# rasoolims/ImageTranslate

Measured on AMD Instinct MI355X. Metric: train tokens/sec (whole node), 6L enc-dec d=512 seq128 b64, 1/2/4/8 GPU, higher is better.
Workload: dtype bf16; 1 GPU; 6L/6L enc-dec d=512 h=8 ff=2048 V=30000, src[64,128] tgt[64,128], synthetic random-token MT; global_batch=64, seq_len=128, parallelism=dp1, distinct_batches=8, directions=2

## Files before the change

imagetranslate_amd/_lib.py:

```python
import ctypes
import os
from ctypes import POINTER, Structure, c_char_p, c_float, c_int, c_int32, c_int64, c_uint64, c_void_p

_HERE = os.path.dirname(os.path.abspath(__file__))
LIB_PATH = os.environ.get("IMT_LIB") or os.path.join(_HERE, "libimt_hip.so")

IMT_F32, IMT_BF16 = 0, 1
IMT_NT, IMT_NN, IMT_TN = 0, 1, 2
IMT_AUX_NONE, IMT_AUX_GELU_FWD, IMT_AUX_DGELU, IMT_AUX_SPLITK_WS = 0, 1, 2, 3


class GemmArgs(Structure):
    _fields_ = [
        ("dtype", c_int32), ("layout", c_int32),
        ("M", c_int32), ("N", c_int32), ("K", c_int32),
        ("A", c_void_p), ("lda", c_int64),
        ("B", c_void_p), ("ldb", c_int64),
        ("C", c_void_p), ("ldc", c_int64),
        ("c_dtype", c_int32), ("accumulate", c_int32),
        ("bias", c_void_p),
        ("resid", c_void_p), ("ldr", c_int64),
        ("aux", c_void_p), ("ldaux", c_int64),
        ("aux_mode", c_int32), ("split_k", c_int32),
        ("alpha", c_float), ("dropout_p", c_float),
# ... 172 lines not shown
        ("dtype", c_int32), ("B", c_int32), ("S", c_int32), ("T", c_int32), ("d", c_int32),
        ("x", c_void_p), ("ldx", c_int64), ("bsx", c_int64),
        ("y", c_void_p), ("ldy", c_int64), ("bsy", c_int64),
        ("xr", c_void_p), ("yr", c_void_p),
        ("min_sim", c_float), ("reserved", c_int32),
        ("link", c_void_p), ("fwd_idx", c_void_p), ("fwd_val", c_void_p), ("bwd_idx", c_void_p), ("bwd_val", c_void_p),
    ]


_P = c_void_p
SIGNATURES = {
    "imt_version": (c_int, []),
    "imt_last_error": (c_char_p, []),
    "imt_gemm": (c_int, [POINTER(GemmArgs), _P]),
    "imt_gemm_grouped_tn": (c_int, [POINTER(GemmArgs), c_int, _P]),
    "imt_gemm_splitk_ws_bytes": (c_int64, []),
    "imt_gemm_bias_residual_ln_supported": (c_int, [c_int, c_int, c_int]),
    "imt_gemm_bias_residual_ln": (c_int, [c_int, _P, c_int64, _P, c_int64, _P, _P, c_int64, _P, _P, _P, _P, c_int64, _P, _P, c_int, c_int,
                                          c_int, c_float, c_float, c_uint64, _P]),
    "imt_colsum": (c_int, [c_int, _P, c_int64, c_int, c_int, _P, _P, _P]),
    "imt_layernorm_fwd": (c_int, [c_int, _P, _P, _P, _P, _P, _P, c_int, c_int, c_float, c_float, c_uint64, _P]),
    "imt_add_layernorm_fwd": (c_int, [c_int, _P, _P, _P, _P, _P, _P, _P, _P, c_int, c_int, c_float, c_float, c_uint64, _P]),
    "imt_embed_ln_fwd": (c_int, [c_int, _P, _P, _P, _P, _P, _P, _P, _P, _P, _P, _P, _P, c_int, c_int, c_int, c_int, c_int, c_int, c_float,
                                 c_float, c_uint64, _P]),
    "imt_layernorm_bwd": (c_int, [c_int, _P, _P, _P, _P, _P, _P, _P, _P, c_int, c_int, c_float, c_uint64, _P, c_float,
                                  c_uint64, _P, _P]),
    "imt_embed_fwd": (c_int, [c_int, _P, _P, _P, _P, _P, _P, _P, c_int, c_int, c_int, c_int, c_int, c_int, _P]),
    "imt_embed_bwd": (c_int, [c_int, _P, _P, _P, _P, _P, _P, _P, c_int, c_int, c_int, c_int64, _P]),
    "imt_attention_fwd": (c_int, [POINTER(AttnArgs), _P]),
    "imt_attention_bwd": (c_int, [POINTER(AttnArgs), _P]),
# ... 38 lines not shown
    "imt_l2_dist": (c_int, [c_int, _P, _P, _P, _P, _P, c_int, c_int64, _P]),
    "imt_sensim_loss": (c_int, [_P, _P, _P, _P, _P, _P, c_int, c_int, c_int, c_int, _P]),
    "imt_pair_dot": (c_int, [_P, _P, _P, c_int64, c_int, _P]),
    "imt_pair_dot_bwd": (c_int, [_P, _P, _P, _P, _P, c_int64, c_int, _P]),
    "imt_proposal_attn_ws_bytes": (c_int64, [c_int64, c_int, c_int, c_int]),
    "imt_proposal_attn_fwd": (c_int, [c_int, _P, _P, _P, _P, _P, _P, _P, _P, _P, c_int64, c_int, c_int, c_int, c_int64, c_int64, c_float, _P]),
    "imt_proposal_attn_bwd": (c_int, [c_int, _P, _P, _P, _P, _P, _P, _P, _P, _P, _P, _P, _P, _P, _P, c_int64, c_int64, c_int, c_int, c_int,
                                      c_int64, c_int64, _P]),
    "imt_comm_unique_id_bytes": (c_int, []),
    "imt_comm_get_unique_id": (c_int, [_P]),
    "imt_comm_init": (c_int, [_P, c_int, c_int, POINTER(c_void_p)]),
    "imt_comm_allreduce": (c_int, [_P, _P, c_int64, c_int, _P]),
    "imt_comm_broadcast": (c_int, [_P, _P, c_int64, c_int, c_int, _P]),
    "imt_comm_destroy": (c_int, [_P]),
    "imt_set_gemm_share_cus": (c_int, [c_int]),
    "imt_debug_spin": (c_int, [c_int, c_int, c_int, c_int64, _P]),
    "imt_abi_sizeof": (c_int, [ctypes.c_char_p]),
    "imt_prof_enable": (c_int, [c_int]),
    "imt_prof_report": (c_int, [POINTER(ProfRow), c_int]),
    "imt_stack_workspace_bytes": (c_int64, [POINTER(StackDesc), c_int, c_int, c_int]),
    "imt_stack_forward": (c_int, [POINTER(StackDesc), POINTER(StackIO), _P, c_int64, _P]),
    "imt_stack_backward": (c_int, [POINTER(StackDesc), POINTER(StackIO), _P, c_int64, c_int, c_int, _P]),
    "imt_attention_decode": (c_int, [POINTER(AttnDecodeArgs), _P]),
    "imt_decode_workspace_bytes": (c_int64, [POINTER(StackDesc), c_int]),
    "imt_decode_self_cache_bytes": (c_int64, [POINTER(StackDesc), c_int, c_int]),
    "imt_decode_cross_bytes": (c_int64, [POINTER(StackDesc), c_int, c_int]),
    "imt_decode_begin": (c_int, [POINTER(StackDesc), _P, c_int, c_int, _P, _P]),
    "imt_decode_step": (c_int, [POINTER(StackDesc), POINTER(DecodeIO), _P, c_int64, _P]),
    "imt_decode_check": (c_int, [POINTER(StackDesc), c_int, _P, _P]),
    "imt_beam_step": (c_int, [POINTER(BeamArgs), _P]),
# ... 48 lines not shown
```

imagetranslate_amd/csrc/common.hpp:

```cpp
#pragma once
#include <hip/hip_runtime.h>
#include <stdint.h>
#include <stdio.h>
#include <string.h>
#include "../../include/imt_hip.h"

typedef __bf16 bf16_t;
typedef __attribute__((ext_vector_type(4))) float f32x4;
typedef __attribute__((ext_vector_type(2))) float f32x2;
typedef __attribute__((ext_vector_type(8))) __bf16 bf16x8;
typedef __attribute__((ext_vector_type(4))) __bf16 bf16x4;
typedef __attribute__((ext_vector_type(2))) __bf16 bf16x2;
typedef __attribute__((ext_vector_type(4))) short s16x4;
typedef __attribute__((ext_vector_type(4))) unsigned int u32x4;
typedef __attribute__((ext_vector_type(2))) unsigned int u32x2;

#define IMT_WAVE 64
#define IMT_DEVICE __device__ __forceinline__

void imt_set_error(const char* fmt, ...);

#define IMT_CHECK_ARG(cond, ...)                       \
  do {                                                  \
    if (!(cond)) {                                      \
// ... 8 lines not shown
    if (e__ != hipSuccess) {                                                 \
      imt_set_error("%s:%d launch failed: %s", __FILE__, __LINE__,           \
                    hipGetErrorString(e__));                                 \
      return IMT_ERR_LAUNCH;                                                 \
    }                                                                        \
  } while (0)

static inline int imt_cdiv(long a, long b) { return (int)((a + b - 1) / b); }
static inline bool imt_ok_dtype(int t) { return t == IMT_F32 || t == IMT_BF16; }
static inline int imt_dtype_bytes(int t) { return t == IMT_BF16 ? 2 : 4; }
static inline int64_t imt_align256(int64_t bytes) { return (bytes + 255) / 256 * 256; }
template <typename T> struct ImtType { typedef T type; };
template <typename F> static inline int imt_by_dtype(int dtype, F&& f) {
  return dtype == IMT_F32 ? f(ImtType<float>()) : f(ImtType<bf16_t>());
}

bool imt_prof_enabled();
const char* imt_prof_intern(const char* kind, int M, int N, int K);
void* imt_prof_begin_launch(const char* kind, double flops, double bytes, hipStream_t st);
void imt_prof_end_launch(void* tok, hipStream_t st);
#include <stdlib.h>
struct ImtTrace {
  static constexpr int MAXB = 4096;
  static constexpr int RING = 64;
  unsigned long long* dev = nullptr;
  const char* kind; int blocks; hipStream_t st;
  struct Slot { const char* kind; int blocks; };
  static Slot* slots() { static Slot s[RING]; return s; }
  static int& count() { static int c = 0; return c; }
  static bool ring() { static const bool r = getenv("IMT_TRACE_RING") != nullptr; return r; }
// ... 239 lines not shown
```

imagetranslate_amd/csrc/gemm.hip:

```cpp
#include <stdlib.h>
#include "mma.hpp"
#include "gemm_xl.hpp"

namespace {

constexpr int BM = 128, BN = 128, NTHREADS = 256;
constexpr int STAGE_BYTES = 2 * TILE_BYTES;


template <typename T, bool KCONTIG> struct Stage : TileGeom<T, KCONTIG> {
  using G = TileGeom<T, KCONTIG>;
  u32x4 r[4];
  IMT_DEVICE void load(const T* __restrict__ base, int64_t ld, int row0, int nrows, int k0, int K) {
    const int tid = threadIdx.x;
#pragma unroll
    for (int i = 0; i < 4; ++i) {
      const int q = i * NTHREADS + tid;
      const int tr = q / G::CPR, c = q % G::CPR;
      int64_t grow, gcol;
      bool ok;
      if (KCONTIG) { grow = row0 + tr; gcol = k0 + c * G::EPC; ok = (grow < nrows) && (gcol < K); }
      else         { grow = k0 + tr;   gcol = row0 + c * G::EPC; ok = (grow < K) && (gcol < nrows); }
      u32x4 v = {0u, 0u, 0u, 0u};
      if (ok) v = *reinterpret_cast<const u32x4*>(base + grow * ld + gcol);
// ... 689 lines not shown
      if (LAYOUT == IMT_TN && do_colsum) cs.flush(smem + half * 16384, ep.a_colsum, m0 + 128 * half, M, alpha, true, ht);
      return;
    }
  }
#pragma unroll 1
  for (int q = 0; q < 4; ++q) {
    const int qm = q >> 1, qn = q & 1;
    const int mq = m0 + 128 * qm, nq = n0 + 128 * qn;
    if (mq >= M || nq >= N) continue;
    if (wmi == qm && (wni >> 1) == qn) epilogue<T, XL_THREADS, true, 128>(acc, smem, mq, nq, 0, wn, M, N, ep, alpha);
    else                               epilogue<T, XL_THREADS, false, 128>(acc, smem, mq, nq, 0, wn, M, N, ep, alpha);
  }
  if (LAYOUT == IMT_TN && do_colsum) cs.flush(smem + half * 16384, ep.a_colsum, m0 + 128 * half, M, alpha, true, ht);
}

constexpr int MAX_GROUP = 8;
struct GroupProblem {
  const void* A; const void* B; float* C; float* a_colsum;
  int64_t lda, ldb, ldc, a_bytes, b_bytes;
  int M, N, K, tile_start;
};
struct GroupArgs { int count; int total_tiles; float alpha; int alpha_pad_order ; GroupProblem p[MAX_GROUP]; };

constexpr int GROUP_NST = 4;
constexpr int GROUP_THREADS = 512;

template <typename T> IMT_DEVICE typename Frag<T>::type ones_frag();
template <> IMT_DEVICE f32x4 ones_frag<float>() { return f32x4{1.f, 1.f, 1.f, 1.f}; }
template <> IMT_DEVICE bf16x8 ones_frag<bf16_t>() {
  const bf16_t o = (bf16_t)1.0f;
  return bf16x8{o, o, o, o, o, o, o, o};
}

template <typename T, bool CS, bool LO>
IMT_DEVICE void grouped_consumer_loop(f32x4 (&acc)[4][4], f32x4 (&bacc)[2], const char* smem, int nt, int wm, int wn) {
  typedef typename Frag<T>::type frag_t;
  constexpr int MPF = sizeof(T) == 2 ? 1 : 4;
// ... 23 lines not shown
#pragma unroll
    for (int i = 0; i < 4; ++i)
#pragma unroll
      for (int j = 0; j < 4; ++j) mma16(acc[i][j], f1b[j], f1a[i]);
    if (CS) { mma16(bacc[0], ones, f1a[LO ? 0 : 2]); mma16(bacc[1], ones, f1a[LO ? 1 : 3]); }
#pragma unroll
    for (int k = 0; k < 16; ++k) {
      __builtin_amdgcn_sched_group_barrier(0x008, MPF, 0);
      __builtin_amdgcn_sched_group_barrier(0x100, 1, 0);
    }
    __builtin_amdgcn_sched_barrier(0);
    cur = nxt;
  }
}

template <typename T>
__global__ __launch_bounds__(GROUP_THREADS) void gemm_grouped_tn_kernel(GroupArgs g) {
  constexpr int BK = TileGeom<T, false>::BK;
  extern __shared__ __attribute__((aligned(16))) char smem[];
  const int bid = (g.alpha_pad_order == 0) ? imt_xcd_block(blockIdx.x, g.total_tiles) : (int)blockIdx.x;
  int pi = 0;
#pragma unroll
  for (int i = 1; i < MAX_GROUP; ++i)
    if (i < g.count && bid >= g.p[i].tile_start) pi = i;
  const GroupProblem& P = g.p[pi];
  const int M = P.M, N = P.N, K = P.K;
  const int nbx = (N + BN - 1) / BN;
  const int local = bid - P.tile_start;
  const int m0 = (local / nbx) * BM, n0 = (local % nbx) * BN;
  const int nt = (K + BK - 1) / BK;
  const int wave = __builtin_amdgcn_readfirstlane(threadIdx.x >> 6);
  const bool consumer = wave < 4;
  const int wm = ((wave & 3) >> 1) * 64, wn = (wave & 1) * 64;

  f32x4 acc[4][4];
#pragma unroll
  for (int i = 0; i < 4; ++i)
#pragma unroll
    for (int j = 0; j < 4; ++j) acc[i][j] = f32x4{0.f, 0.f, 0.f, 0.f};
  f32x4 bacc[2] = {f32x4{0.f, 0.f, 0.f, 0.f}, f32x4{0.f, 0.f, 0.f, 0.f}};
  const bool do_colsum = P.a_colsum && n0 == 0;

  if (!consumer) {
    Dma<T, false> da; Dma<T, false> db;
// ... 441 lines not shown
  int splits = a->split_k > 1 ? a->split_k : 1, kps = a->K;
  if (splits > 1) {
    IMT_CHECK_ARG(a->c_dtype == IMT_F32 && !a->bias && !a->resid && a->aux_mode == IMT_AUX_NONE && a->dropout_p == 0.f,
                  "imt_gemm: split_k supports only fp32 atomic accumulation without epilogue");
    kps = imt_cdiv(imt_cdiv(a->K, splits), f.bk) * f.bk;
    splits = imt_cdiv(a->K, kps);
  }
  if (a->aux_mode != IMT_AUX_NONE) IMT_CHECK_ARG(a->aux != nullptr, "imt_gemm: aux_mode needs aux");
  const GemmSwitches& sw = gemm_switches();
  const bool linear_epilogue = a->aux_mode == IMT_AUX_NONE && a->dropout_p == 0.f && !a->a_colsum;
  if (a->force_general == 0 && splits == 1 && a->layout != IMT_TN && a->K % f.bk != 0 && a->K / f.bk >= 16 && linear_epilogue) return run_ragged_k(a, f, stream);
  if (const int S = splitk_ws_splits(a, f, sw, splits); S > 1) return run_splitk_ws(a, f, S, stream);
  return run_single(a, f, sw, splits, kps, stream);
}

extern "C" int imt_gemm_grouped_tn(const imt_gemm_args* list, int count, void* stream) {
  IMT_CHECK_ARG(list && count >= 0, "imt_gemm_grouped_tn: bad args");
  if (count == 0) return IMT_OK;
  hipStream_t st = reinterpret_cast<hipStream_t>(stream);
  bool ok = count <= MAX_GROUP;
  const int dtype = list[0].dtype;
  const int bk = (dtype == IMT_BF16) ? 64 : 32, es = imt_dtype_bytes(dtype), al = (dtype == IMT_BF16) ? 8 : 4;
  int tiles = 0;
  for (int i = 0; i < count && ok; ++i) {
    const imt_gemm_args& a = list[i];
    ok = a.dtype == dtype && a.layout == IMT_TN && a.c_dtype == IMT_F32 && !a.bias && !a.resid && a.aux_mode == IMT_AUX_NONE &&
         a.dropout_p == 0.f && !a.alpha_dev && a.alpha == list[0].alpha && a.A && a.B && a.C && a.M > 0 && a.N > 0 &&
         a.K / bk >= 2 && a.lda % al == 0 && a.ldb % al == 0 && a.M % al == 0 && a.N % al == 0 && a.ldc % 4 == 0 &&
         (((uintptr_t)a.A | (uintptr_t)a.B) & 15) == 0 && (int64_t)a.K * a.lda * es < (1ll << 31) &&
         (int64_t)a.K * a.ldb * es < (1ll << 31);
    tiles += imt_cdiv(a.M, BM) * imt_cdiv(a.N, BN);
  }
  if (!ok || tiles > 640) {
    for (int i = 0; i < count; ++i) {
      int rc = imt_gemm(&list[i], stream);
      if (rc != IMT_OK) return rc;
    }
    return IMT_OK;
  }
  GroupArgs g;
  memset(&g, 0, sizeof(g));
  g.count = count; g.alpha = list[0].alpha; g.alpha_pad_order = gemm_switches().grouped_plain_order ? 1 : 0;
  int start = 0;
  double flops = 0, bytes = 0;
  for (int i = 0; i < count; ++i) {
    const imt_gemm_args& a = list[i];
    GroupProblem& P = g.p[i];
    P.A = a.A; P.B = a.B; P.C = reinterpret_cast<float*>(a.C); P.a_colsum = a.a_colsum;
    P.lda = a.lda; P.ldb = a.ldb; P.ldc = a.ldc;
    P.a_bytes = view_bytes(a.K, a.lda, a.M, es); P.b_bytes = view_bytes(a.K, a.ldb, a.N, es);
    P.M = a.M; P.N = a.N; P.K = a.K; P.tile_start = start;
    start += imt_cdiv(a.M, BM) * imt_cdiv(a.N, BN);
    flops += 2.0 * a.M * a.N * a.K;
    bytes += ((double)a.M + a.N) * a.K * es + 4.0 * a.M * a.N;
  }
  g.total_tiles = start;
  static const bool once_f32 = allow_lds(gemm_grouped_tn_kernel<float>, GROUP_NST * STAGE_BYTES), once_bf16 = allow_lds(gemm_grouped_tn_kernel<bf16_t>, GROUP_NST * STAGE_BYTES);
  ImtProfScope prof(dtype == IMT_BF16 ? "gemm_bf16_tn_grouped" : "gemm_f32_tn_grouped", flops, bytes, st);
  auto kern = (dtype == IMT_F32) ? gemm_grouped_tn_kernel<float> : gemm_grouped_tn_kernel<bf16_t>;
  hipLaunchKernelGGL(kern, dim3(start), dim3(GROUP_THREADS), GROUP_NST * STAGE_BYTES, st, g);
  IMT_CHECK_LAUNCH();
  return IMT_OK;
}
```

imagetranslate_amd/csrc/model.hip:

```cpp
#include "common.hpp"
#include "decode_fused.hpp"

namespace {

struct Carver {
  char* base; int64_t off;
  explicit Carver(void* b) : base(reinterpret_cast<char*>(b)), off(0) {}
  void* take(int64_t bytes) {
    void* p = base ? base + off : nullptr;
    off += (bytes + 255) & ~(int64_t)255;
    return p;
  }
};

struct AttnWs {
  void* qkv;
  void* kv;
  int64_t kv_ld;
  void* ctx;
  float* lse;
  void* pre_ln;
  float* mean; float* rstd;
  void* out;
};
// ... 2 lines not shown
  void* z; void* h;
  void* pre_ln2; float* mean2; float* rstd2;
  void* out;
};
struct StackWs {
  void* emb_sum; float* emb_mean; float* emb_rstd; void* x0;
  LayerWs* layers;
  void* d_run;
  void* dpre[3]; void* ddrop[3];
  void* d_ctx;
  void* d_ff;
  void* d_qkv;
  void* d_q;
  void* d_kv;
  void* d_emb;
  struct Scratch { void* dpre[3]; void* ddrop[3]; void* d_ctx; void* d_ff; void* d_qkv; void* d_q; void* d_kv; } scr[2];
  void use_scratch(int l) {
    const Scratch& z = scr[l & 1];
    for (int i = 0; i < 3; ++i) { dpre[i] = z.dpre[i]; ddrop[i] = z.ddrop[i]; }
    d_ctx = z.d_ctx; d_ff = z.d_ff; d_qkv = z.d_qkv; d_q = z.d_q; d_kv = z.d_kv;
  }
  void* kv_all; void* d_kv_all;
  float* delta;
  float* ln_partial;
  float* ln_site(int site, int d) const { return ln_partial + (int64_t)site * IMT_LN_BWD_WS_FLOATS(d); }
  void* splitk; int64_t splitk_bytes;
  int64_t bytes;
};

constexpr int MAX_LAYERS = 64;

int64_t kv_w_off(const imt_stack_desc* m, const imt_layer_desc& p) { return p.cross_kv_w >= 0 ? p.cross_kv_w : p.cross_attn.qkv_w + (int64_t)m->d * m->d; }
int64_t kv_b_off(const imt_stack_desc* m, const imt_layer_desc& p) { return p.cross_kv_b >= 0 ? p.cross_kv_b : p.cross_attn.qkv_b + m->d; }
// ... 29 lines not shown
    AttnWs& x = L.cross;
    memset(&x, 0, sizeof(x));
    if (m->is_decoder && m->layers[l].cross_attn.qkv_w >= 0) {
      x.qkv = c.take(N * d * es); x.ctx = c.take(N * d * es);
      if (batched) { x.kv = w.kv_all ? (void*)((char*)w.kv_all + (int64_t)l * 2 * d * es) : nullptr; x.kv_ld = L2d; }
      else { x.kv = c.take(Nk * 2 * d * es); x.kv_ld = 2 * d; }
      x.lse = (float*)c.take((int64_t)B * m->heads * T * 4);
      x.pre_ln = c.take(N * d * es); x.mean = (float*)c.take(N * 4); x.rstd = (float*)c.take(N * 4);
      x.out = c.take(N * d * es);
    }
    L.z = c.take(N * ff * es); L.h = c.take(N * ff * es);
    L.pre_ln2 = c.take(N * d * es); L.mean2 = (float*)c.take(N * 4); L.rstd2 = (float*)c.take(N * 4);
    L.out = c.take(N * d * es);
  }
  w.d_run = c.take(N * d * es);
  for (int k = 0; k < 2; ++k) {
    StackWs::Scratch& z = w.scr[k];
    for (int i = 0; i < 3; ++i) { z.dpre[i] = c.take(N * d * es); z.ddrop[i] = c.take(N * d * es); }
    z.d_ctx = c.take(N * d * es);
    z.d_ff = c.take(N * ff * es);
    z.d_qkv = c.take(N * 3 * d * es);
    z.d_q = c.take(N * d * es);
    z.d_kv = c.take((Nk > 0 ? Nk : 1) * 2 * d * es);
  }
  w.use_scratch(0);
  w.d_emb = c.take(N * d * es);
  w.delta = (float*)c.take((int64_t)B * m->heads * T * 4);
  w.ln_partial = (float*)c.take((int64_t)(3 * m->n_layers + 1) * IMT_LN_BWD_WS_FLOATS(d) * 4);
  w.splitk_bytes = ((N + 127) / 128) * ((d + 127) / 128) <= 128 ? imt_gemm_splitk_ws_bytes() : 0;
  w.splitk = w.splitk_bytes ? c.take(w.splitk_bytes) : nullptr;
  w.bytes = c.off;
// ... 46 lines not shown
                                     pre_ln, out, N, mean, rstd, M, N, K, c.m->ln_eps, drop_p, seed, c.st);
  imt_gemm_args a;
  memset(&a, 0, sizeof(a));
  a.dtype = c.dtype; a.layout = IMT_NT; a.M = M; a.N = N; a.K = K;
  a.A = x; a.lda = ldx; a.B = c.P(w_off); a.ldb = K; a.C = pre_ln; a.ldc = N; a.c_dtype = c.dtype;
  a.bias = b_off >= 0 ? c.P(b_off) : nullptr;
  a.resid = resid; a.ldr = N; a.aux_mode = IMT_AUX_NONE; a.split_k = 1; a.alpha = 1.f;
  a.dropout_p = drop_p; a.dropout_seed = seed;
  a.ln_gamma = c.P(g_off); a.ln_beta = c.P(beta_off); a.ln_out = out; a.ld_ln = N; a.ln_mean = mean; a.ln_rstd = rstd;
  a.ln_eps = c.m->ln_eps;
  a.splitk_ws = c.splitk; a.splitk_ws_bytes = c.splitk_bytes;
  return imt_gemm(&a, c.st);
}

struct DeferredDW {
  imt_gemm_args list[8];
  int n = 0;
  void add(const Ctx& c, const void* dy, int64_t lddy, const void* x, int64_t ldx, int M, int N, int K, int64_t w_off, int64_t b_off) {
    imt_gemm_args& a = list[n++];
    memset(&a, 0, sizeof(a));
    a.dtype = c.dtype; a.layout = IMT_TN; a.M = N; a.N = K; a.K = M;
    a.A = dy; a.lda = lddy; a.B = x; a.ldb = ldx; a.C = c.G(w_off); a.ldc = K; a.c_dtype = IMT_F32; a.alpha = 1.f;
    a.split_k = 1; a.accumulate = 1;
    a.a_colsum = b_off >= 0 ? c.G(b_off) : nullptr;
    const int tiles = imt_cdiv(N, 128) * imt_cdiv(K, 128);
    int sk = 1;
    while (sk < 8 && tiles * sk * 2 <= 256 && M / (sk * 2) >= 512) sk *= 2;
    if (M % (c.dtype == IMT_BF16 ? 64 : 32) != 0) { a.split_k = sk; a.accumulate = (sk == 1); }
  }
  int flush(hipStream_t st) {
    const int rc = n ? imt_gemm_grouped_tn(list, n, st) : IMT_OK;
    n = 0;
// ... 198 lines not shown
  IMT_CHECK_ARG(0 <= layer_lo && layer_lo <= layer_hi && layer_hi <= m->n_layers, "stack_backward: bad layer range");
  Ctx c{m, (hipStream_t)stream, m->dtype, imt_dtype_bytes(m->dtype)};
  c.splitk = w.splitk; c.splitk_bytes = w.splitk_bytes;
  const int B = io->B, T = io->T, N = B * T, d = m->d;
  const bool training = io->training != 0;
  const uint64_t seed = io->dropout_seed;
  const MaskSet self_ms{io->key_mask, io->query_mask, io->mask3d, io->causal};
  const MaskSet cross_ms{io->enc_mask, nullptr, nullptr, 0};
  const void* dy = (layer_hi == m->n_layers) ? io->d_out : w.d_run;
  const bool batched = cross_kv_batched(m);
  DeferredDW dw;
  const int64_t lnf = IMT_LN_BWD_WS_FLOATS(d);
  if (layer_hi > layer_lo) (void)hipMemsetAsync(w.ln_site(3 * layer_lo, d), 0, (size_t)(3 * (layer_hi - layer_lo)) * lnf * 4, c.st);
  if (layer_lo == 0) (void)hipMemsetAsync(w.ln_site(3 * m->n_layers, d), 0, (size_t)lnf * 4, c.st);
  static const bool side_env = !(getenv("IMT_DW_SIDE_STREAM") && atoi(getenv("IMT_DW_SIDE_STREAM")) == 0);
  const bool side = side_env && !imt_prof_enabled() && layer_lo == 0 && layer_hi == m->n_layers && m->n_layers >= 2 && g_side.init();
  int last_side = -1;
  for (int l = layer_hi - 1; l >= layer_lo; --l) {
    const imt_layer_desc& p = m->layers[l];
    LayerWs& L = layers[l];
    w.use_scratch(l);
    if (side && l + 2 < layer_hi) (void)hipStreamWaitEvent(c.st, g_side.done[l + 2], 0);
    if (l == m->n_layers - 1) L.out = io->out;
    const bool has_cross = m->is_decoder && p.cross_attn.qkv_w >= 0;
    const void* x_in = (l == 0) ? w.x0 : (const void*)layers[l - 1].out;
    const void* a_self = L.self_attn.out;
    const void* a_ffn_in = has_cross ? L.cross.out : a_self;
    RC(ffn_bwd(c, p, L, w, dw, a_ffn_in, N, training, seed, l, dy));
    if (has_cross) {
      const bool first_cross = (l == m->n_layers - 1);
      void* dkv_l = batched ? offp(w.d_kv_all, (int64_t)l * 2 * d, c.es) : nullptr;
      RC(attn_block_bwd(c, p.cross_attn, L.cross, w, dw, 1, a_self, B, T, io->enc_states, io->Tk, cross_ms, training, seed, l, 4, w.d_run,
                        io->d_enc_states, first_cross ? 0 : 1, kv_w_off(m, p), kv_b_off(m, p), dkv_l));
    }
    RC(attn_block_bwd(c, p.self_attn, L.self_attn, w, dw, 2, x_in, B, T, nullptr, 0, self_ms, training, seed, l, 0, w.d_run, nullptr, 0));
    if (side) {
      (void)hipEventRecord(g_side.ready[l], c.st);
      (void)hipStreamWaitEvent(g_side.st, g_side.ready[l], 0);
      RC(dw.flush(g_side.st));
      (void)hipEventRecord(g_side.done[l], g_side.st);
      last_side = l;
    } else {
      RC(dw.flush(c.st));
    }
    dy = w.d_run;
  }
  if (layer_lo == 0 && batched) {
    const int Nk = B * io->Tk;
    const int L2d = m->n_layers * 2 * d;
    if (io->d_enc_states)
      RC(linear_bwd_input(c, w.d_kv_all, L2d, Nk, L2d, m->layers[0].cross_kv_w, d, io->d_enc_states, d, nullptr, 0, nullptr, IMT_AUX_NONE, 0));
  }
  if (layer_lo == 0) {
    const void* dy0 = (m->n_layers == 0) ? io->d_out : dy;
    RC(imt_layernorm_bwd(c.dtype, dy0, w.emb_sum, c.P(m->emb_ln_g), w.emb_mean, w.emb_rstd, w.d_emb, c.G(m->emb_ln_g), c.G(m->emb_ln_b), N, d,
                         training ? m->hidden_dropout : 0.f, site_seed(seed, 1000, 0), nullptr, 0.f, 0, w.ln_site(3 * m->n_layers, d), c.st));
    RC(imt_embed_bwd(c.dtype, io->ids, io->pos_ids, io->type_ids, w.d_emb, c.G(m->emb_word), c.G(m->emb_pos), c.G(m->emb_type), N, T, d,
                     m->pad_id, c.st));
// ... 203 lines not shown
```

imagetranslate_amd/hip_ops.py:

```python
import ctypes
import os
import math

import torch

from . import _lib as L
from ._lib import IMT_AUX_DGELU, IMT_AUX_GELU_FWD, IMT_AUX_NONE, IMT_AUX_SPLITK_WS, IMT_BF16, IMT_F32, IMT_NN, IMT_NT, IMT_TN


def dt(t: torch.Tensor) -> int:
    if t.dtype == torch.float32:
        return IMT_F32
    if t.dtype == torch.bfloat16:
        return IMT_BF16
    raise TypeError("imagetranslate_amd supports float32 and bfloat16 tensors, got %s" % t.dtype)


def _stream():
    return ctypes.c_void_p(torch.cuda.current_stream().cuda_stream)


def _p(t):
    return None if t is None else ctypes.c_void_p(t.data_ptr())

# ... 73 lines not shown


def splitk_workspace(device):
    key = (device.type, device.index)
    ws = _SPLITK_WS.get(key)
    if ws is None:
        ws = torch.empty(int(L.load().imt_gemm_splitk_ws_bytes()) // 4, device=device, dtype=torch.float32)
        _SPLITK_WS[key] = ws
    return ws


def dw_split_k(rows: int, N: int, K: int, rows_per_split: int) -> int:
    return max(1, min(rows // rows_per_split, 512 // max(1, ((N + 127) // 128) * ((K + 127) // 128))))


def gemm_grouped_tn(problems):
    arr = (L.GemmArgs * len(problems))()
    for i, pr in enumerate(problems):
        arr[i] = gemm(pr["A"], pr["B"], IMT_TN, out=pr["out"], accumulate=True, a_colsum=pr.get("a_colsum"), _launch=False)
    L.check(L.load().imt_gemm_grouped_tn(arr, len(problems), _stream()), "imt_gemm_grouped_tn")


def gemm_bias_residual_ln(x, w, bias, resid, gamma, beta, eps=1e-12, dropout_p=0.0, dropout_seed=0, want_pre_ln=True):
    _req_cuda(x, w, bias, resid, gamma, beta)
    M, K = x.shape
    N = w.shape[0]
    assert w.shape[1] == K
    out = torch.empty((M, N), device=x.device, dtype=x.dtype)
    pre = torch.empty((M, N), device=x.device, dtype=x.dtype) if want_pre_ln else None
    mean = torch.empty(M, device=x.device, dtype=torch.float32)
    rstd = torch.empty(M, device=x.device, dtype=torch.float32)
    L.check(L.load().imt_gemm_bias_residual_ln(dt(x), _p(x), _rowmajor(x), _p(w), _rowmajor(w), _p(bias), _p(resid),
                                               _rowmajor(resid) if resid is not None else 0, _p(gamma), _p(beta), _p(pre), _p(out), N,
                                               _p(mean), _p(rstd), M, N, K, eps, dropout_p, dropout_seed, _stream()),
            "imt_gemm_bias_residual_ln")
# ... 775 lines not shown
```

include/imt_hip.h:

```cpp
#ifndef IMT_HIP_H
#define IMT_HIP_H
#include <stdint.h>
#ifdef __cplusplus
extern "C" {
#endif

#define IMT_OK 0
#define IMT_ERR_BAD_ARG (-1)
#define IMT_ERR_UNSUPPORTED (-2)
#define IMT_ERR_LAUNCH (-3)

#define IMT_F32 0
#define IMT_BF16 1

int imt_version(void);
const char* imt_last_error(void);

int imt_abi_sizeof(const char* struct_name);

typedef struct imt_prof_row {
  char kind[48];
  int64_t launches;
  double total_ms;
  double flops;
// ... 30 lines not shown
  const float* alpha_dev;
  float* a_colsum;
  int32_t force_general;
  int32_t force_pipeline;
  const void* ln_gamma; const void* ln_beta;
  void* ln_out; int64_t ld_ln;
  float* ln_mean; float* ln_rstd;
  int32_t* ln_tickets;
  float ln_eps;
  int32_t reserved_ln;
  void* splitk_ws; int64_t splitk_ws_bytes;
} imt_gemm_args;
int64_t imt_gemm_splitk_ws_bytes(void);
int imt_gemm(const imt_gemm_args* a, void* stream);
int imt_gemm_grouped_tn(const imt_gemm_args* list, int count, void* stream);

int imt_gemm_bias_residual_ln_supported(int dtype, int N, int K);
int imt_gemm_bias_residual_ln(int dtype, const void* x, int64_t ldx, const void* w, int64_t ldw, const void* bias,
                              const void* resid, int64_t ldr, const void* gamma, const void* beta, void* pre_ln, void* out,
                              int64_t ldo, float* mean, float* rstd, int M, int N, int K, float eps, float dropout_p,
                              uint64_t dropout_seed, void* stream);

int imt_colsum(int dtype, const void* X, int64_t ldx, int M, int N, float* out, const float* scale_dev, void* stream);

int imt_layernorm_fwd(int dtype, const void* x, const void* gamma, const void* beta, void* y, float* mean,
                      float* rstd, int rows, int d, float eps, float dropout_p, uint64_t dropout_seed,
                      void* stream);
int imt_add_layernorm_fwd(int dtype, const void* x, const void* resid, const void* gamma, const void* beta, void* sum_out,
                          void* y, float* mean, float* rstd, int rows, int d, float eps, float dropout_p,
                          uint64_t dropout_seed, void* stream);
// ... 106 lines not shown
  int32_t* fwd_idx; float* fwd_val;
  int32_t* bwd_idx; float* bwd_val;
} imt_align_args;
int imt_align_supported(int dtype, int d);
int imt_align_pairs(const imt_align_args* a, void* stream);
int imt_scaled_sum(const float* x, int n, float scale, float* out, void* stream);

int imt_comm_unique_id_bytes(void);
int imt_comm_get_unique_id(void* host_id_out);
int imt_comm_init(const void* host_unique_id, int world_size, int rank, void** comm_out);
int imt_comm_allreduce(void* comm, void* buf, int64_t count, int dtype, void* stream);
int imt_comm_broadcast(void* comm, void* buf, int64_t count, int dtype, int root, void* stream);
int imt_comm_destroy(void* comm);

int imt_set_gemm_share_cus(int share_cus);

#define IMT_SUMSQ_WS_FLOATS 1024
int imt_sumsq(const float* g, int64_t n, float* out, float* partial_ws, void* stream);
int imt_clip_adam(float* p, float* g, float* m, float* v, void* p_bf16, int64_t n, const float* sumsq,
                  float max_norm, float grad_scale, float lr, float beta1, float beta2, float eps, int64_t step,
                  int zero_grad, void* stream);
int imt_clip_scale(float* g, int64_t n, const float* sumsq, float max_norm, float grad_scale, void* stream);
int imt_cast_f32_to_bf16(const float* src, void* dst, int64_t n, void* stream);
int imt_gated_mix(int dtype, const void* a, const void* b, const void* gate, void* out, int64_t rows, int d,
                  void* stream);
int imt_add_rows_dropout(int in_dtype, const void* x, int out_dtype, void* out, const void* add, int64_t rows, int d,
                         int period, float dropout_p, uint64_t dropout_seed, void* stream);

#define IMT_OBJ_FEAT_DIM 1024
#define IMT_OBJ_LABELS 91
// ... 234 lines not shown
```

Baseline: 1.120 million tokens/s.

## Add tall 256-row grouped weight-grad GEMM and pair layers' deferred dW flushes

Adds a 256-row-tile variant of the grouped TN weight-gradient GEMM with a 6-stage slab DMA pipeline. It is chosen when the group has enough tiles to fill most CUs. The backward pass now holds one layer's deferred dW GEMMs and flushes them together with the next layer's, doubling group size, and scratch buffers grow from 2 to 4 so the side stream can lag further behind. The intent is fewer, larger, better-occupied grouped GEMM launches with more A/B reuse per tile. The cost is extra workspace memory, larger kernel args (MAX_GROUP 16), and delayed overlap of dW work on the side stream.

Measured after the change: 1.161 million tokens/s (median of 6 runs). +3.7%, better.

```diff
diff --git a/imagetranslate_amd/_lib.py b/imagetranslate_amd/_lib.py
--- a/imagetranslate_amd/_lib.py
+++ b/imagetranslate_amd/_lib.py
@@ -210,6 +210,7 @@
     "imt_last_error": (c_char_p, []),
     "imt_gemm": (c_int, [POINTER(GemmArgs), _P]),
     "imt_gemm_grouped_tn": (c_int, [POINTER(GemmArgs), c_int, _P]),
+    "imt_gemm_grouped_tile_order": (c_int, [POINTER(c_int), POINTER(c_int), c_int, c_int, POINTER(c_int), c_int]),
     "imt_gemm_splitk_ws_bytes": (c_int64, []),
     "imt_gemm_bias_residual_ln_supported": (c_int, [c_int, c_int, c_int]),
     "imt_gemm_bias_residual_ln": (c_int, [c_int, _P, c_int64, _P, c_int64, _P, _P, c_int64, _P, _P, _P, _P, c_int64, _P, _P, c_int, c_int,
@@ -278,6 +279,7 @@
     "imt_comm_broadcast": (c_int, [_P, _P, c_int64, c_int, c_int, _P]),
     "imt_comm_destroy": (c_int, [_P]),
     "imt_set_gemm_share_cus": (c_int, [c_int]),
+    "imt_set_gemm_grouped_tall_min_tiles": (c_int, [c_int]),
     "imt_debug_spin": (c_int, [c_int, c_int, c_int, c_int64, _P]),
     "imt_abi_sizeof": (c_int, [ctypes.c_char_p]),
     "imt_prof_enable": (c_int, [c_int]),
diff --git a/imagetranslate_amd/csrc/common.hpp b/imagetranslate_amd/csrc/common.hpp
--- a/imagetranslate_amd/csrc/common.hpp
+++ b/imagetranslate_amd/csrc/common.hpp
@@ -46,6 +46,8 @@
 template <typename F> static inline int imt_by_dtype(int dtype, F&& f) {
   return dtype == IMT_F32 ? f(ImtType<float>()) : f(ImtType<bf16_t>());
 }
+
+bool imt_gemm_grouped_tall(const imt_gemm_args* list, int count);
 
 bool imt_prof_enabled();
 const char* imt_prof_intern(const char* kind, int M, int N, int K);
diff --git a/imagetranslate_amd/csrc/gemm.hip b/imagetranslate_amd/csrc/gemm.hip
--- a/imagetranslate_amd/csrc/gemm.hip
+++ b/imagetranslate_amd/csrc/gemm.hip
@@ -727,13 +727,29 @@
   if (LAYOUT == IMT_TN && do_colsum) cs.flush(smem + half * 16384, ep.a_colsum, m0 + 128 * half, M, alpha, true, ht);
 }
 
-constexpr int MAX_GROUP = 8;
+constexpr int MAX_GROUP = 16;
 struct GroupProblem {
   const void* A; const void* B; float* C; float* a_colsum;
   int64_t lda, ldb, ldc, a_bytes, b_bytes;
-  int M, N, K, tile_start;
+  int M, N, K;
 };
-struct GroupArgs { int count; int total_tiles; float alpha; int alpha_pad_order ; GroupProblem p[MAX_GROUP]; };
+struct GroupGrid { int rows, cols, tile_start; };
+struct GroupTile { int problem, row, col; };
+struct GroupArgs { int count; int total_tiles; float alpha; int plain_order ; GroupGrid grid[MAX_GROUP]; GroupProblem p[MAX_GROUP]; };
+
+__host__ __device__ inline GroupTile grouped_tile(int wg, int total, int count, const GroupGrid* grid, bool plain) {
+  int pos = wg;
+  if (!plain) {
+    const int q = total >> 3, r = total & 7, xcd = wg & 7, idx = wg >> 3;
+    pos = (xcd < r ? xcd * (q + 1) : r * (q + 1) + (xcd - r) * q) + idx;
+  }
+  int pi = 0;
+#pragma unroll
+  for (int i = 1; i < MAX_GROUP; ++i)
+    if (i < count && pos >= grid[i].tile_start) pi = i;
+  const int local = pos - grid[pi].tile_start, cols = grid[pi].cols;
+  return GroupTile{pi, local / cols, local % cols};
+}
 
 constexpr int GROUP_NST = 4;
 constexpr int GROUP_THREADS = 512;
@@ -787,20 +803,161 @@
   }
 }
 
+constexpr int SLAB_PART = TILE_BYTES / 2;
+constexpr int TALL_SLAB = 3 * SLAB_PART;
+constexpr int TALL_NST = 6;
+
+template <typename T> struct SlabDma {
+  typedef TileGeom<T, false> G;
+  __amdgpu_buffer_rsrc_t ra, rb;
+  int va[2], vb[2], kadv_a, kadv_b, wv;
+  IMT_DEVICE void init(const GroupProblem& P, int m0, int n0, int wave) {
+    ra = __builtin_amdgcn_make_buffer_rsrc(const_cast<void*>(P.A), 0, (int)P.a_bytes, 0x00020000);
+    rb = __builtin_amdgcn_make_buffer_rsrc(const_cast<void*>(P.B), 0, (int)P.b_bytes, 0x00020000);
+    const int lane = threadIdx.x & 63;
+    wv = wave;
+#pragma unroll
+    for (int i = 0; i < 2; ++i) {
+      const int q = 64 * (4 * i + wave) + lane;
+      const int tr = q / G::CPR, pc = q % G::CPR;
+      const int c = pc ^ swz<G::RB>(tr);
+      va[i] = (int)((((int64_t)tr) * P.lda + m0 + c * G::EPC) * (int64_t)sizeof(T));
+      vb[i] = (int)((((int64_t)tr) * P.ldb + n0 + c * G::EPC) * (int64_t)sizeof(T));
+    }
+    kadv_a = (int)(Frag<T>::KSTEP * P.lda * (int64_t)sizeof(T));
+    kadv_b = (int)(Frag<T>::KSTEP * P.ldb * (int64_t)sizeof(T));
+  }
+  IMT_DEVICE void issue(char* slab, int t) const {
+    const int wave = __builtin_amdgcn_readfirstlane(wv);
+#pragma unroll
+    for (int i = 0; i < 2; ++i) {
+      char* dst = slab + (4 * i + wave) * 1024;
+      const int oa = va[i] + t * kadv_a, ob = vb[i] + t * kadv_b;
+      __builtin_amdgcn_raw_ptr_buffer_load_lds(ra, (__attribute__((address_space(3))) void*)dst, 16, oa, 0, 0, 0);
+      __builtin_amdgcn_raw_ptr_buffer_load_lds(ra, (__attribute__((address_space(3))) void*)(dst + SLAB_PART), 16, oa + 128 * (int)sizeof(T), 0, 0, 0);
+      __builtin_amdgcn_raw_ptr_buffer_load_lds(rb, (__attribute__((address_space(3))) void*)(dst + 2 * SLAB_PART), 16, ob, 0, 0, 0);
+    }
+  }
+};
+IMT_DEVICE void slab_wait_newer(int newer) {
+  if (newer >= 4)      asm volatile("s_waitcnt vmcnt(24)" ::: "memory");
+  else if (newer == 3) asm volatile("s_waitcnt vmcnt(18)" ::: "memory");
+  else if (newer == 2) asm volatile("s_waitcnt vmcnt(12)" ::: "memory");
+  else if (newer == 1) asm volatile("s_waitcnt vmcnt(6)" ::: "memory");
+  else                 asm volatile("s_waitcnt vmcnt(0)" ::: "memory");
+}
+
+template <typename T, bool CS, bool LO>
+IMT_DEVICE void grouped_consumer_loop_tall(f32x4 (&acc)[8][4], f32x4 (&bacc)[4], const char* smem, int ns, int wmi, int wn) {
+  typedef typename Frag<T>::type frag_t;
+  typedef TileGeom<T, false> G;
+  constexpr int MPF = sizeof(T) == 2 ? 1 : 4;
+  constexpr int RPF = sizeof(T) == 2 ? 2 : 4;
+  frag_t fa[8], fb[4];
+  const frag_t ones = ones_frag<T>();
+  asm volatile("s_barrier" ::: "memory");
+#pragma unroll
+  for (int j = 0; j < 4; ++j) fb[j] = KStrided<T, G::RB>::load(smem + 2 * SLAB_PART, 0, wn + 16 * j);
+#pragma unroll
+  for (int i = 0; i < 8; ++i) fa[i] = KStrided<T, G::RB>::load(smem + wmi * SLAB_PART, 0, 16 * i);
+  int cur = 0;
+  for (int t = 0; t < ns; ++t) {
+    asm volatile("s_barrier" ::: "memory");
+    const int nxt = (cur + 1 == TALL_NST) ? 0 : cur + 1;
+    const char* sn = smem + nxt * TALL_SLAB;
+    frag_t nb[4];
+#pragma unroll
+    for (int j = 0; j < 4; ++j) nb[j] = KStrided<T, G::RB>::load(sn + 2 * SLAB_PART, 0, wn + 16 * j);
+#pragma unroll
+    for (int i = 0; i < 8; ++i) {
+#pragma unroll
+      for (int j = 0; j < 4; ++j) mma16(acc[i][j], fb[j], fa[i]);
+      if (CS && (LO ? i < 4 : i >= 4)) mma16(bacc[i & 3], ones, fa[i]);
+      fa[i] = KStrided<T, G::RB>::load(sn + wmi * SLAB_PART, 0, 16 * i);
+    }
+#pragma unroll
+    for (int j = 0; j < 4; ++j) fb[j] = nb[j];
+#pragma unroll
+    for (int i = 0; i < 4; ++i) {
+      __builtin_amdgcn_sched_group_barrier(0x008, (CS && LO ? 5 : 4) * MPF, 0);
+      __builtin_amdgcn_sched_group_barrier(0x100, 3 * RPF / 2, 0);
+    }
+#pragma unroll
+    for (int i = 4; i < 8; ++i) {
+      __builtin_amdgcn_sched_group_barrier(0x008, (CS && !LO ? 5 : 4) * MPF, 0);
+      __builtin_amdgcn_sched_group_barrier(0x100, 3 * RPF / 2, 0);
+    }
+    __builtin_amdgcn_sched_barrier(0);
+    cur = nxt;
+  }
+}
+
 template <typename T>
+IMT_DEVICE void grouped_tall_tile(const GroupArgs& g, const GroupProblem& P, int m0, int n0, char* smem) {
+  const int M = P.M, N = P.N, K = P.K;
+  const int ns = (K + Frag<T>::KSTEP - 1) / Frag<T>::KSTEP;
+  const int wave = __builtin_amdgcn_readfirstlane(threadIdx.x >> 6);
+  const bool consumer = wave < 4;
+  const int wmi = (wave & 3) >> 1, wn = (wave & 1) * 64;
+  f32x4 acc[8][4];
+  xl_zero(acc);
+  f32x4 bacc[4];
+#pragma unroll
+  for (int k = 0; k < 4; ++k) bacc[k] = f32x4{0.f, 0.f, 0.f, 0.f};
+  const bool do_colsum = P.a_colsum && n0 == 0;
+  if (!consumer) {
+    SlabDma<T> dma;
+    dma.init(P, m0, n0, wave - 4);
+#pragma unroll
+    for (int s0 = 0; s0 < TALL_NST - 1; ++s0)
+      if (s0 < ns) dma.issue(smem + s0 * TALL_SLAB, s0);
+    slab_wait_newer(min(TALL_NST - 2, ns - 1));
+    asm volatile("s_barrier" ::: "memory");
+    int cur = 0;
+    for (int t = 0; t < ns; ++t) {
+      slab_wait_newer(max(0, min(TALL_NST - 3, ns - 2 - t)));
+      asm volatile("s_barrier" ::: "memory");
+      if (t + TALL_NST - 1 < ns) dma.issue(smem + ((cur == 0) ? TALL_NST - 1 : cur - 1) * TALL_SLAB, t + TALL_NST - 1);
+      cur = (cur + 1 == TALL_NST) ? 0 : cur + 1;
+    }
+  } else {
+    if (!do_colsum)   grouped_consumer_loop_tall<T, false, false>(acc, bacc, smem, ns, wmi, wn);
+    else if (wn == 0) grouped_consumer_loop_tall<T, true, true>(acc, bacc, smem, ns, wmi, wn);
+    else              grouped_consumer_loop_tall<T, true, false>(acc, bacc, smem, ns, wmi, wn);
+  }
+  EpiParams ep;
+  ep.C = P.C; ep.ldc = P.ldc; ep.c_f32 = 1; ep.accumulate = 1;
+  ep.bias = nullptr; ep.resid = nullptr; ep.ldr = 0; ep.aux = nullptr; ep.ldaux = 0; ep.aux_mode = IMT_AUX_NONE;
+  ep.atomic = 0; ep.alpha = g.alpha; ep.alpha_dev = nullptr; ep.inv_keep = 1.f; ep.drop_thresh = 0; ep.seed = 0;
+  ep.a_colsum = P.a_colsum; ep.dbg = 0; ep.trace = nullptr;
+#pragma unroll 1
+  for (int q = 0; q < 2; ++q) {
+    const int mq = m0 + 128 * q;
+    if (mq >= M) continue;
+    if (consumer && wmi == q) epilogue<T, 512, true, 128>(acc, smem, mq, n0, 0, wn, M, N, ep, g.alpha);
+    else                      epilogue<T, 512, false, 128>(acc, smem, mq, n0, 0, wn, M, N, ep, g.alpha);
+  }
+  if (do_colsum && consumer && (threadIdx.x & 63) < 16) {
+    const int mb = m0 + 128 * wmi + ((wn == 0) ? 0 : 64) + (threadIdx.x & 15);
+#pragma unroll
+    for (int k = 0; k < 4; ++k)
+      if (mb + 16 * k < M) atomicAdd(P.a_colsum + mb + 16 * k, bacc[k][0] * g.alpha);
+  }
+}
+
+template <typename T, int TM>
 __global__ __launch_bounds__(GROUP_THREADS) void gemm_grouped_tn_kernel(GroupArgs g) {
   constexpr int BK = TileGeom<T, false>::BK;
   extern __shared__ __attribute__((aligned(16))) char smem[];
-  const int bid = (g.alpha_pad_order == 0) ? imt_xcd_block(blockIdx.x, g.total_tiles) : (int)blockIdx.x;
-  int pi = 0;
-#pragma unroll
-  for (int i = 1; i < MAX_GROUP; ++i)
-    if (i < g.count && bid >= g.p[i].tile_start) pi = i;
-  const GroupProblem& P = g.p[pi];
+  if constexpr (TM == 256) {
+    const GroupTile tile = grouped_tile(blockIdx.x, g.total_tiles, g.count, g.grid, g.plain_order != 0);
+    grouped_tall_tile<T>(g, g.p[tile.problem], tile.row * 256, tile.col * BN, smem);
+    return;
+  }
+  const GroupTile tile = grouped_tile(blockIdx.x, g.total_tiles, g.count, g.grid, g.plain_order != 0);
+  const GroupProblem& P = g.p[tile.problem];
   const int M = P.M, N = P.N, K = P.K;
-  const int nbx = (N + BN - 1) / BN;
-  const int local = bid - P.tile_start;
-  const int m0 = (local / nbx) * BM, n0 = (local % nbx) * BN;
+  const int m0 = tile.row * BM, n0 = tile.col * BN;
   const int nt = (K + BK - 1) / BK;
   const int wave = __builtin_amdgcn_readfirstlane(threadIdx.x >> 6);
   const bool consumer = wave < 4;
@@ -1272,6 +1429,49 @@
   return run_single(a, f, sw, splits, kps, stream);
 }
 
+constexpr int GROUP_CUS = 256;
+constexpr int GROUP_MAX_TILES = 640;
+static int g_tall_min_tiles = 0;
+static bool grouped_tall(const imt_gemm_args* list, int count, int cus) {
+  int tiles = 0;
+  for (int i = 0; i < count; ++i) {
+    if (list[i].M % 256 != 0) return false;
+    tiles += (list[i].M / 256) * imt_cdiv(list[i].N, BN);
+  }
+  return 2 * tiles <= GROUP_MAX_TILES && (g_tall_min_tiles > 0 ? tiles >= g_tall_min_tiles : 4 * tiles >= 3 * cus);
+}
+extern "C" int imt_set_gemm_grouped_tall_min_tiles(int min_tiles) {
+  const int prev = g_tall_min_tiles;
+  return g_tall_min_tiles = min_tiles > 0 ? min_tiles : 0, prev;
+}
+bool imt_gemm_grouped_tall(const imt_gemm_args* list, int count) { return count >= 1 && count <= MAX_GROUP && grouped_tall(list, count, GROUP_CUS); }
+
+static int grouped_grids(const int* rows, const int* cols, int count, GroupGrid* grid) {
+  int start = 0;
+  for (int i = 0; i < count; ++i) {
+    grid[i] = GroupGrid{rows[i], cols[i], start};
+    start += rows[i] * cols[i];
+  }
+  return start;
+}
+
+extern "C" int imt_gemm_grouped_tile_order(const int* tile_rows, const int* tile_cols, int count, int plain, int* order, int order_tiles) {
+  IMT_CHECK_ARG(tile_rows && tile_cols && order && count >= 1 && count <= MAX_GROUP, "imt_gemm_grouped_tile_order: bad args");
+  int64_t total = 0;
+  for (int i = 0; i < count; ++i) {
+    IMT_CHECK_ARG(tile_rows[i] >= 1 && tile_cols[i] >= 1 && tile_rows[i] <= 640 && tile_cols[i] <= 640, "imt_gemm_grouped_tile_order: bad tile grid");
+    total += (int64_t)tile_rows[i] * tile_cols[i];
+  }
+  IMT_CHECK_ARG(total <= GROUP_MAX_TILES && total == order_tiles, "imt_gemm_grouped_tile_order: the group has %d tiles (at most 640), order_tiles is %d", (int)total, order_tiles);
+  GroupGrid grid[MAX_GROUP];
+  grouped_grids(tile_rows, tile_cols, count, grid);
+  for (int w = 0; w < order_tiles; ++w) {
+    const GroupTile t = grouped_tile(w, order_tiles, count, grid, plain != 0);
+    order[3 * w] = t.problem; order[3 * w + 1] = t.row; order[3 * w + 2] = t.col;
+  }
+  return IMT_OK;
+}
+
 extern "C" int imt_gemm_grouped_tn(const imt_gemm_args* list, int count, void* stream) {
   IMT_CHECK_ARG(list && count >= 0, "imt_gemm_grouped_tn: bad args");
   if (count == 0) return IMT_OK;
@@ -1289,17 +1489,19 @@
          (int64_t)a.K * a.ldb * es < (1ll << 31);
     tiles += imt_cdiv(a.M, BM) * imt_cdiv(a.N, BN);
   }
-  if (!ok || tiles > 640) {
+  if (!ok || tiles > GROUP_MAX_TILES) {
     for (int i = 0; i < count; ++i) {
       int rc = imt_gemm(&list[i], stream);
       if (rc != IMT_OK) return rc;
     }
     return IMT_OK;
   }
+  const bool tall = grouped_tall(list, count, GROUP_CUS);
+  const int tm = tall ? 256 : BM;
   GroupArgs g;
   memset(&g, 0, sizeof(g));
-  g.count = count; g.alpha = list[0].alpha; g.alpha_pad_order = gemm_switches().grouped_plain_order ? 1 : 0;
-  int start = 0;
+  g.count = count; g.alpha = list[0].alpha; g.plain_order = gemm_switches().grouped_plain_order ? 1 : 0;
+  int rows[MAX_GROUP], cols[MAX_GROUP];
   double flops = 0, bytes = 0;
   for (int i = 0; i < count; ++i) {
     const imt_gemm_args& a = list[i];
@@ -1307,16 +1509,22 @@
     P.A = a.A; P.B = a.B; P.C = reinterpret_cast<float*>(a.C); P.a_colsum = a.a_colsum;
     P.lda = a.lda; P.ldb = a.ldb; P.ldc = a.ldc;
     P.a_bytes = view_bytes(a.K, a.lda, a.M, es); P.b_bytes = view_bytes(a.K, a.ldb, a.N, es);
-    P.M = a.M; P.N = a.N; P.K = a.K; P.tile_start = start;
-    start += imt_cdiv(a.M, BM) * imt_cdiv(a.N, BN);
+    P.M = a.M; P.N = a.N; P.K = a.K;
+    rows[i] = imt_cdiv(a.M, tm); cols[i] = imt_cdiv(a.N, BN);
     flops += 2.0 * a.M * a.N * a.K;
     bytes += ((double)a.M + a.N) * a.K * es + 4.0 * a.M * a.N;
   }
-  g.total_tiles = start;
-  static const bool once_f32 = allow_lds(gemm_grouped_tn_kernel<float>, GROUP_NST * STAGE_BYTES), once_bf16 = allow_lds(gemm_grouped_tn_kernel<bf16_t>, GROUP_NST * STAGE_BYTES);
+  const int start = g.total_tiles = grouped_grids(rows, cols, count, g.grid);
+  static const bool once_f32 = allow_lds(gemm_grouped_tn_kernel<float, 128>, GROUP_NST * STAGE_BYTES), once_bf16 = allow_lds(gemm_grouped_tn_kernel<bf16_t, 128>, GROUP_NST * STAGE_BYTES);
+  static const bool tall_f32 = allow_lds(gemm_grouped_tn_kernel<float, 256>, TALL_NST * TALL_SLAB), tall_bf16 = allow_lds(gemm_grouped_tn_kernel<bf16_t, 256>, TALL_NST * TALL_SLAB);
   ImtProfScope prof(dtype == IMT_BF16 ? "gemm_bf16_tn_grouped" : "gemm_f32_tn_grouped", flops, bytes, st);
-  auto kern = (dtype == IMT_F32) ? gemm_grouped_tn_kernel<float> : gemm_grouped_tn_kernel<bf16_t>;
-  hipLaunchKernelGGL(kern, dim3(start), dim3(GROUP_THREADS), GROUP_NST * STAGE_BYTES, st, g);
+  if (tall) {
+    auto kern = (dtype == IMT_F32) ? gemm_grouped_tn_kernel<float, 256> : gemm_grouped_tn_kernel<bf16_t, 256>;
+    hipLaunchKernelGGL(kern, dim3(start), dim3(GROUP_THREADS), TALL_NST * TALL_SLAB, st, g);
+  } else {
+    auto kern = (dtype == IMT_F32) ? gemm_grouped_tn_kernel<float, 128> : gemm_grouped_tn_kernel<bf16_t, 128>;
+    hipLaunchKernelGGL(kern, dim3(start), dim3(GROUP_THREADS), GROUP_NST * STAGE_BYTES, st, g);
+  }
   IMT_CHECK_LAUNCH();
   return IMT_OK;
 }
diff --git a/imagetranslate_amd/csrc/model.hip b/imagetranslate_amd/csrc/model.hip
--- a/imagetranslate_amd/csrc/model.hip
+++ b/imagetranslate_amd/csrc/model.hip
@@ -40,9 +40,10 @@
   void* d_q;
   void* d_kv;
   void* d_emb;
-  struct Scratch { void* dpre[3]; void* ddrop[3]; void* d_ctx; void* d_ff; void* d_qkv; void* d_q; void* d_kv; } scr[2];
+  static constexpr int N_SCRATCH = 4;
+  struct Scratch { void* dpre[3]; void* ddrop[3]; void* d_ctx; void* d_ff; void* d_qkv; void* d_q; void* d_kv; } scr[N_SCRATCH];
   void use_scratch(int l) {
-    const Scratch& z = scr[l & 1];
+    const Scratch& z = scr[l % N_SCRATCH];
     for (int i = 0; i < 3; ++i) { dpre[i] = z.dpre[i]; ddrop[i] = z.ddrop[i]; }
     d_ctx = z.d_ctx; d_ff = z.d_ff; d_qkv = z.d_qkv; d_q = z.d_q; d_kv = z.d_kv;
   }
@@ -102,7 +103,7 @@
     L.out = c.take(N * d * es);
   }
   w.d_run = c.take(N * d * es);
-  for (int k = 0; k < 2; ++k) {
+  for (int k = 0; k < StackWs::N_SCRATCH; ++k) {
     StackWs::Scratch& z = w.scr[k];
     for (int i = 0; i < 3; ++i) { z.dpre[i] = c.take(N * d * es); z.ddrop[i] = c.take(N * d * es); }
     z.d_ctx = c.take(N * d * es);
@@ -179,8 +180,14 @@
 }
 
 struct DeferredDW {
-  imt_gemm_args list[8];
+  imt_gemm_args list[16];
   int n = 0;
+  bool hold_for_pair() const {
+    if (n == 0 || 2 * n > 16) return false;
+    imt_gemm_args two[16];
+    for (int i = 0; i < n; ++i) two[i] = two[n + i] = list[i];
+    return imt_gemm_grouped_tall(two, 2 * n);
+  }
   void add(const Ctx& c, const void* dy, int64_t lddy, const void* x, int64_t ldx, int M, int N, int K, int64_t w_off, int64_t b_off) {
     imt_gemm_args& a = list[n++];
     memset(&a, 0, sizeof(a));
@@ -409,13 +416,16 @@
   if (layer_hi > layer_lo) (void)hipMemsetAsync(w.ln_site(3 * layer_lo, d), 0, (size_t)(3 * (layer_hi - layer_lo)) * lnf * 4, c.st);
   if (layer_lo == 0) (void)hipMemsetAsync(w.ln_site(3 * m->n_layers, d), 0, (size_t)lnf * 4, c.st);
   static const bool side_env = !(getenv("IMT_DW_SIDE_STREAM") && atoi(getenv("IMT_DW_SIDE_STREAM")) == 0);
-  const bool side = side_env && !imt_prof_enabled() && layer_lo == 0 && layer_hi == m->n_layers && m->n_layers >= 2 && g_side.init();
+  const bool whole = layer_lo == 0 && layer_hi == m->n_layers && m->n_layers >= 2;
+  const bool side = side_env && !imt_prof_enabled() && whole && g_side.init();
+  const bool pairs = whole && !imt_prof_enabled();
   int last_side = -1;
+  int held = -1;
   for (int l = layer_hi - 1; l >= layer_lo; --l) {
     const imt_layer_desc& p = m->layers[l];
     LayerWs& L = layers[l];
     w.use_scratch(l);
-    if (side && l + 2 < layer_hi) (void)hipStreamWaitEvent(c.st, g_side.done[l + 2], 0);
+    if (side && l + StackWs::N_SCRATCH < layer_hi) (void)hipStreamWaitEvent(c.st, g_side.done[l + StackWs::N_SCRATCH], 0);
     if (l == m->n_layers - 1) L.out = io->out;
     const bool has_cross = m->is_decoder && p.cross_attn.qkv_w >= 0;
     const void* x_in = (l == 0) ? w.x0 : (const void*)layers[l - 1].out;
@@ -429,14 +439,20 @@
                         io->d_enc_states, first_cross ? 0 : 1, kv_w_off(m, p), kv_b_off(m, p), dkv_l));
     }
     RC(attn_block_bwd(c, p.self_attn, L.self_attn, w, dw, 2, x_in, B, T, nullptr, 0, self_ms, training, seed, l, 0, w.d_run, nullptr, 0));
-    if (side) {
+    const bool first_of_pair = pairs && held < 0 && l > layer_lo && dw.hold_for_pair();
+    if (first_of_pair) {
+      held = l;
+    } else if (side) {
       (void)hipEventRecord(g_side.ready[l], c.st);
       (void)hipStreamWaitEvent(g_side.st, g_side.ready[l], 0);
       RC(dw.flush(g_side.st));
       (void)hipEventRecord(g_side.done[l], g_side.st);
+      if (held >= 0) (void)hipEventRecord(g_side.done[held], g_side.st);
+      held = -1;
       last_side = l;
     } else {
       RC(dw.flush(c.st));
+      held = -1;
     }
     dy = w.d_run;
   }
diff --git a/imagetranslate_amd/hip_ops.py b/imagetranslate_amd/hip_ops.py
--- a/imagetranslate_amd/hip_ops.py
+++ b/imagetranslate_amd/hip_ops.py
@@ -1,3 +1,4 @@
+import contextlib
 import ctypes
 import os
 import math
@@ -111,11 +112,30 @@
     return max(1, min(rows // rows_per_split, 512 // max(1, ((N + 127) // 128) * ((K + 127) // 128))))
 
 
-def gemm_grouped_tn(problems):
+@contextlib.contextmanager
+def grouped_tall_min_tiles(min_tiles):
+    prev = L.load().imt_set_gemm_grouped_tall_min_tiles(int(min_tiles))
+    try:
+        yield
+    finally:
+        L.load().imt_set_gemm_grouped_tall_min_tiles(prev)
+
+
+def gemm_grouped_tn(problems, tile_rows=0):
     arr = (L.GemmArgs * len(problems))()
     for i, pr in enumerate(problems):
         arr[i] = gemm(pr["A"], pr["B"], IMT_TN, out=pr["out"], accumulate=True, a_colsum=pr.get("a_colsum"), _launch=False)
-    L.check(L.load().imt_gemm_grouped_tn(arr, len(problems), _stream()), "imt_gemm_grouped_tn")
+    with grouped_tall_min_tiles({128: 1 << 30, 256: 1}[tile_rows]) if tile_rows else contextlib.nullcontext():
+        L.check(L.load().imt_gemm_grouped_tn(arr, len(problems), _stream()), "imt_gemm_grouped_tn")
+
+
+def grouped_tile_order(grids, plain=False):
+    n = len(grids)
+    total = sum(r * c for r, c in grids)
+    rows, cols = (ctypes.c_int * n)(*[g[0] for g in grids]), (ctypes.c_int * n)(*[g[1] for g in grids])
+    order = (ctypes.c_int * (3 * total))()
+    L.check(L.load().imt_gemm_grouped_tile_order(rows, cols, n, int(plain), order, total), "imt_gemm_grouped_tile_order")
+    return [(order[3 * w], order[3 * w + 1], order[3 * w + 2]) for w in range(total)]
 
 
 def gemm_bias_residual_ln(x, w, bias, resid, gamma, beta, eps=1e-12, dropout_p=0.0, dropout_seed=0, want_pre_ln=True):
diff --git a/include/imt_hip.h b/include/imt_hip.h
--- a/include/imt_hip.h
+++ b/include/imt_hip.h
@@ -68,6 +68,7 @@
 int64_t imt_gemm_splitk_ws_bytes(void);
 int imt_gemm(const imt_gemm_args* a, void* stream);
 int imt_gemm_grouped_tn(const imt_gemm_args* list, int count, void* stream);
+int imt_gemm_grouped_tile_order(const int* tile_rows, const int* tile_cols, int count, int plain, int* order, int order_tiles);
 
 int imt_gemm_bias_residual_ln_supported(int dtype, int N, int K);
 int imt_gemm_bias_residual_ln(int dtype, const void* x, int64_t ldx, const void* w, int64_t ldw, const void* bias,
@@ -204,6 +205,7 @@
 int imt_comm_destroy(void* comm);
 
 int imt_set_gemm_share_cus(int share_cus);
+int imt_set_gemm_grouped_tall_min_tiles(int min_tiles);
 
 #define IMT_SUMSQ_WS_FLOATS 1024
 int imt_sumsq(const float* g, int64_t n, float* out, float* partial_ws, void* stream);
```
